# Thefefe/orbit

Hardware: AMD Instinct MI355X
Metric: meshlets_culled_per_sec (higher is better)
Workload: dtype f32

## Files before the change

orbit_amd/csrc/block_pretest.h:

```cpp
#pragma once
#include <math.h>
#include <stdint.h>
#include <string.h>

#if defined(__HIPCC__) || defined(__CUDACC__)
#define ORBIT_BLK_FN __host__ __device__ inline
#else
#define ORBIT_BLK_FN inline
#endif

namespace orbit {

ORBIT_BLK_FN uint32_t blk_bits(float f) {
    uint32_t u;
    __builtin_memcpy(&u, &f, 4);
    return u;
}
ORBIT_BLK_FN float blk_float(uint32_t u) {
    float f;
    __builtin_memcpy(&f, &u, 4);
    return f;
}
ORBIT_BLK_FN uint32_t blk_up16(float x) { return (blk_bits(x) + 0xFFFFu) >> 16; }

struct BlockBound {
    float cx, cy, cz;
    uint32_t packed;
    float rc;
    float r_max;
    uint32_t valid;
    uint32_t pad_;
};
static_assert(sizeof(BlockBound) == 32, "BlockBound layout");

ORBIT_BLK_FN BlockBound block_bound_unpack(float cx, float cy, float cz, uint32_t packed) {
    BlockBound b;
    b.cx = cx, b.cy = cy, b.cz = cz, b.packed = packed;
    b.rc = blk_float(packed & 0xFFFF0000u);
    b.r_max = blk_float(packed << 16);
    b.valid = (packed >> 16) != 0u ? 1u : 0u;
    b.pad_ = 0u;
    return b;
}

struct BlockRecord {
    float gx, gy, gz, dk;
    float sigma;
    float bk;
    float rr;
    uint32_t flags;
};
static_assert(sizeof(BlockRecord) == 32, "BlockRecord layout");
constexpr uint32_t kBlkSparse = 1u;
constexpr uint32_t kBlkInside = 2u;

constexpr float kBlkEps = 0x1p-18f;
constexpr float kBlkSlack = 1.0f + 0x1p-10f;
constexpr float kBlkUp = 1.0f + 0x1p-20f;
constexpr float kBlkTiny = 0x1p-80f;
constexpr float kBlkHuge = 0x1p60f;
#ifndef ORBIT_BLK_RATIO
#define ORBIT_BLK_RATIO 8.0f
#endif

ORBIT_BLK_FN float blk_max(float a, float b) { return a > b ? a : b; }

ORBIT_BLK_FN BlockBound block_bound_finish(float cx, float cy, float cz, float dist_max, float r_max, float r_min, bool finite) {
    BlockBound b;
    b.cx = cx, b.cy = cy, b.cz = cz;
    b.rc = dist_max * kBlkUp + 0x1p-60f;
    b.r_max = r_max;
    const bool ok = finite && r_min >= 0.0f && b.rc < kBlkHuge && r_max < kBlkHuge && fabsf(cx) < kBlkHuge &&
                    fabsf(cy) < kBlkHuge && fabsf(cz) < kBlkHuge;
    b.valid = ok ? 1u : 0u;
    b.packed = ok ? (blk_up16(b.rc) << 16 | blk_up16(r_max)) : 0u;
    b.pad_ = 0u;
    return b;
}
ORBIT_BLK_FN float block_dist(float cx, float cy, float cz, float x, float y, float z) {
    const float dx = x - cx, dy = y - cy, dz = z - cz;
    return sqrtf(fmaf(dz, dz, fmaf(dy, dy, dx * dx)));
}

ORBIT_BLK_FN BlockBound block_bound_of(const float *spheres, uint32_t n) {
    const float inf = INFINITY;
    float lo[3] = {inf, inf, inf}, hi[3] = {-inf, -inf, -inf}, r_max = 0.0f, r_min = 0.0f;
    bool finite = true;
    for (uint32_t i = 0; i < n; i++) {
        const float *s = spheres + 4 * i;
        for (int k = 0; k < 3; k++) lo[k] = fminf(lo[k], s[k]), hi[k] = fmaxf(hi[k], s[k]);
        r_max = fmaxf(r_max, s[3]), r_min = fminf(r_min, s[3]);
        finite = finite && isfinite(s[0]) && isfinite(s[1]) && isfinite(s[2]) && isfinite(s[3]);
    }
    const float cx = 0.5f * lo[0] + 0.5f * hi[0], cy = 0.5f * lo[1] + 0.5f * hi[1], cz = 0.5f * lo[2] + 0.5f * hi[2];
    float dist = 0.0f;
    for (uint32_t i = 0; i < n; i++) dist = fmaxf(dist, block_dist(cx, cy, cz, spheres[4 * i], spheres[4 * i + 1], spheres[4 * i + 2]));
    return block_bound_finish(cx, cy, cz, dist, r_max, r_min, finite);
}

ORBIT_BLK_FN BlockRecord block_record_setup(const float *m, bool affine, float scale, const BlockBound &b, bool covered,
                                            const float *planes, uint32_t n_planes, float ratio = ORBIT_BLK_RATIO) {
    BlockRecord o;
    const float Cx = b.cx, Cy = b.cy, Cz = b.cz;
    const float dx = fmaf(m[8], Cz, fmaf(m[4], Cy, fmaf(m[0], Cx, m[12])));
    const float dy = fmaf(m[9], Cz, fmaf(m[5], Cy, fmaf(m[1], Cx, m[13])));
    const float dz = fmaf(m[10], Cz, fmaf(m[6], Cy, fmaf(m[2], Cx, m[14])));
    const float aCx = fabsf(Cx), aCy = fabsf(Cy), aCz = fabsf(Cz);
    const float apx = fmaf(fabsf(m[8]), aCz, fmaf(fabsf(m[4]), aCy, fmaf(fabsf(m[0]), aCx, fabsf(m[12]))));
    const float apy = fmaf(fabsf(m[9]), aCz, fmaf(fabsf(m[5]), aCy, fmaf(fabsf(m[1]), aCx, fabsf(m[13]))));
    const float apz = fmaf(fabsf(m[10]), aCz, fmaf(fabsf(m[6]), aCy, fmaf(fabsf(m[2]), aCx, fabsf(m[14]))));
    const float g00 = fmaf(m[2], m[2], fmaf(m[1], m[1], m[0] * m[0]));
    const float g11 = fmaf(m[6], m[6], fmaf(m[5], m[5], m[4] * m[4]));
    const float g22 = fmaf(m[10], m[10], fmaf(m[9], m[9], m[8] * m[8]));
    const float g01 = fabsf(fmaf(m[2], m[6], fmaf(m[1], m[5], m[0] * m[4])));
    const float g02 = fabsf(fmaf(m[2], m[10], fmaf(m[1], m[9], m[0] * m[8])));
    const float g12 = fabsf(fmaf(m[6], m[10], fmaf(m[5], m[9], m[4] * m[8])));
    const float s2 = blk_max(g00 + g01 + g02, blk_max(g11 + g01 + g12, g22 + g02 + g12));
    const float sigma = sqrtf(s2) * (1.0f + 0x1p-16f) + 0x1p-60f;
    const float ap = (blk_max(apx, blk_max(apy, apz)) + 2.0f * sigma * b.rc) * kBlkUp;
    const float rcp = fmaf(kBlkEps, ap, sigma * b.rc * kBlkUp);
    const float D = sqrtf(fmaf(dz, dz, fmaf(dy, dy, dx * dx)));
    const float gx = fmaf(m[2], dz, fmaf(m[1], dy, m[0] * dx));
    const float gy = fmaf(m[6], dz, fmaf(m[5], dy, m[4] * dx));
    const float gz = fmaf(m[10], dz, fmaf(m[9], dy, m[8] * dx));
    const float kf = 0x1.020408p-7f;
    const float mag = ap + D + rcp;
    o.gx = gx * kf, o.gy = gy * kf, o.gz = gz * kf, o.dk = D * kf;
    o.sigma = sigma;
    o.bk = kf * fmaf(kBlkEps, mag, rcp) * kBlkSlack;
    o.rr = b.r_max * scale * kBlkSlack + kBlkTiny;
    bool sparse = affine && covered && b.valid != 0u && D > ratio * rcp && D > 0x1p-40f && mag < kBlkHuge &&
                  sigma < 0x1p40f && o.rr < kBlkHuge && scale >= 0.0f;
    bool inside = sparse;
    for (uint32_t i = 0; i < n_planes; i++) {
        const float nx = planes[4 * i], ny = planes[4 * i + 1], nz = planes[4 * i + 2], w = planes[4 * i + 3];
        const float nn = sqrtf(fmaf(nz, nz, fmaf(ny, ny, nx * nx))) * kBlkUp + kBlkTiny;
        const float dist = fmaf(nz, dz, fmaf(ny, dy, fmaf(nx, dx, w))) - nn * rcp;
        const float margin = fmaf(kBlkEps, fmaf(nn, mag, fabsf(w)), kBlkTiny);
        inside = inside && dist > margin;
    }
    o.flags = (sparse ? kBlkSparse : 0u) | (inside ? kBlkInside : 0u);
    return o;
}

ORBIT_BLK_FN void block_pretest_terms(const BlockRecord &r, uint32_t cone, float &s0, float &band) {
    const float ax = (float)(int)(int8_t)(cone & 0xFFu), ay = (float)(int)(int8_t)((cone >> 8) & 0xFFu);
    const float az = (float)(int)(int8_t)((cone >> 16) & 0xFFu), co = (float)(int)(int8_t)(cone >> 24);
    s0 = fmaf(r.gx, ax, fmaf(r.gy, ay, fmaf(r.gz, az, -(co * r.dk))));
    const float a1 = fabsf(ax) + fabsf(ay) + fabsf(az);
    band = fmaf(r.bk, fmaf(r.sigma, a1, fabsf(co)), kBlkTiny);
}
ORBIT_BLK_FN bool block_cone_culls(const BlockRecord &r, float s0, float band) { return s0 >= band + r.rr; }
ORBIT_BLK_FN bool block_cone_keeps(float s0, float band) { return s0 < -band; }
ORBIT_BLK_FN uint32_t block_pretest(const BlockRecord &r, uint32_t cone) {
    float s0, band;
    block_pretest_terms(r, cone, s0, band);
    return block_cone_culls(r, s0, band) ? 1u : (block_cone_keeps(s0, band) ? 2u : 0u);
}

}
```

orbit_amd/csrc/meshlet_eval_blocks.hip:

```cpp
#include "block_pretest.h"
#include "meshlet_common.h"

namespace orbit {

namespace {

constexpr int kBkWaves = 4;
constexpr int kBkWavesPerSimd = 5;
constexpr uint32_t kBkRing = 512, kBkFlush = 64;

struct __attribute__((aligned(16))) BlockTileLds {
    BlockRecord r[kTileRecords];
};
struct CandRing {
    uint16_t code[kBkRing];
};
struct RingState {
    uint32_t head = 0, count = 0;
    uint32_t total = 0;
};

__device__ __forceinline__ bool row_is_sparse(const WaveTileLds &L, int r) {
    const uint32_t w = reinterpret_cast<const uint32_t *>(&L.pad_)[0];
    return (((uint32_t)__builtin_amdgcn_readfirstlane((int)w) >> (2 * r)) & 1u) != 0u;
}

struct BoundRegs {
    float4 q;
};
__device__ __forceinline__ BoundRegs blk_load_bound(const MeshletCullParams &p, const BlockBound *blk, const uint4 &rec, int lane) {
    const int src_lane = (lane & 15) * 4;
    const uint32_t y = (uint32_t)__shfl((int)rec.y, src_lane, 64), z = (uint32_t)__shfl((int)rec.z, src_lane, 64);
    const uint32_t rel = y - p.ms.first;
    BoundRegs b;
    const bool covered = lane < (int)kTileRecords && z != 0u && (y & 31u) == 0u && rel < p.ms.count && z <= p.ms.count - rel;
    const float4 *src = covered ? reinterpret_cast<const float4 *>(blk + (y >> 5)) : reinterpret_cast<const float4 *>(p.zero_page);
    b.q = src[0];
    return b;
}

__device__ __forceinline__ void blk_setup(const MeshletCullParams &p, WaveTileLds &L, BlockTileLds &B, const PlaneLds &P,
                                          const BoundRegs &bb, int lane) {
    uint32_t flags = 0u;
    if (lane < (int)kTileRecords) {
        const RecordLds &R = L.r[lane];
        float m[16];
#pragma unroll
        for (int c = 0; c < 4; c++) {
            const float4 col = R.mcol[c];
            m[4 * c] = col.x, m[4 * c + 1] = col.y, m[4 * c + 2] = col.z, m[4 * c + 3] = col.w;
        }
        const BlockBound b = block_bound_unpack(bb.q.x, bb.q.y, bb.q.z, __float_as_uint(bb.q.w));
        const uint32_t aw = reinterpret_cast<const uint32_t *>(&L.affine_rows)[lane >> 3];
        const bool affine = ((aw >> (8 * ((lane >> 1) & 3))) & 1u) != 0u;
        BlockRecord o = block_record_setup(m, affine, R.scale, b, true, reinterpret_cast<const float *>(P.plane),
                                           min(p.ci.cull_plane_count, (uint32_t)ORBIT_MAX_CULL_PLANES));
        if (R.rec.z == 0u) o.flags = kBlkSparse;
        B.r[lane] = o;
        flags = o.flags;
    }
    uint64_t m = __ballot((flags & kBlkSparse) != 0u);
    m &= m >> 1;
    if (lane == 0) L.pad_ = m & 0x5555ull;
    __builtin_amdgcn_fence(__ATOMIC_RELEASE, "wavefront");
    __builtin_amdgcn_wave_barrier();
    __builtin_amdgcn_fence(__ATOMIC_ACQUIRE, "wavefront");
}

struct PipeRegs {
    uint32_t v[10];
};

__device__ __forceinline__ bool tile_is_sparse(const WaveTileLds &L) {
    const uint32_t w = reinterpret_cast<const uint32_t *>(&L.pad_)[0];
    return (uint32_t)__builtin_amdgcn_readfirstlane((int)w) == 0x5555u;
}

template <int R>
__device__ __forceinline__ void blk_row_load(const MeshletCullParams &p, const WaveTileLds &L, bool sparse, int lane,
                                             uint32_t *v, const StreamRsrc &SR) {
    const uint32_t half = lane >> 5, ml = lane & 31;
    const uint4 rec = L.r[2 * R + half].rec;
    const bool active = ml < rec.z;
    const uint32_t rel = rec.y + ml - SR.first;
    const bool in = active & (rel < SR.count);
    if (active & !in) latch_status(p.status, ORBIT_E_RANGE);
    const uint32_t i = in ? rel : kNoOffset >> 4;
    const uint32_t is = sparse ? kNoOffset >> 4 : i;
    const auto sp = __builtin_amdgcn_raw_buffer_load_b128(SR.sphere, is << 4, 0, ORBIT_EVAL_LOAD_AUX);
    v[4] = __builtin_amdgcn_raw_buffer_load_b32(SR.cone, i << 2, 0, ORBIT_EVAL_LOAD_AUX);
    v[0] = sp[0], v[1] = sp[1], v[2] = sp[2], v[3] = sp[3];
}

__device__ __forceinline__ void blk_tile_load(const MeshletCullParams &p, const WaveTileLds &L, int lane, uint32_t *v,
                                              const StreamRsrc &SR) {
    const uint32_t half = lane >> 5, ml = lane & 31;
    bool bad = false;
#pragma unroll
    for (int r = 0; r < (int)kTileRows; r++) {
        const uint4 rec = L.r[2 * r + half].rec;
        const bool active = ml < rec.z;
        const uint32_t rel = rec.y + ml - SR.first;
        const bool in = active & (rel < SR.count);
        bad |= active & !in;
        const uint32_t i = in ? rel : kNoOffset >> 4;
        v[r] = __builtin_amdgcn_raw_buffer_load_b32(SR.cone, i << 2, 0, ORBIT_EVAL_LOAD_AUX);
    }
    if (bad) latch_status(p.status, ORBIT_E_RANGE);
}

template <int R>
__device__ __forceinline__ uint32_t blk_row_dense(const MeshletCullParams &p, WaveTileLds &L, const PlaneLds &P, int lane,
                                                  const uint32_t *v, uint32_t total) {
    RowRegs<1> t;
    t.a[0] = make_uint4(v[0], v[1], v[2], v[3]);
    t.b[0] = make_uint4(v[4], 0u, 0u, 0u);
    t.prev[0] = 0u;
    return rows_eval<0, 0, R, 1, true>(p, L, P, nullptr, lane, t, total, nullptr);
}

template <int R>
__device__ __forceinline__ void blk_row_eval(WaveTileLds &L, const BlockTileLds &B, CandRing &ring, int lane,
                                             uint32_t cone, RingState &rs) {
    const uint32_t half = lane >> 5;
    const BlockRecord br = B.r[2 * R + half];
    float s0, band;
    block_pretest_terms(br, cone, s0, band);
    const uint64_t culled = ballot(block_cone_culls(br, s0, band));
    const uint64_t kept = ballot(block_cone_keeps(s0, band)) & ballot((br.flags & kBlkInside) != 0u);
    const uint32_t lo = (uint32_t)__builtin_amdgcn_readfirstlane((int)L.r[2 * R].amask.x);
    const uint32_t hi = (uint32_t)__builtin_amdgcn_readfirstlane((int)L.r[2 * R + 1].amask.x);
    const uint64_t allow = (uint64_t)hi << 32 | lo;
    const uint64_t draw = allow & kept & ~culled;
    const uint64_t cand = allow & ~culled & ~kept;
    if (lane == 0) L.draw_mask[R] = draw;
    rs.total += (uint32_t)__popcll(draw);
    if (lane_of(cand)) ring.code[(rs.head + rs.count + lane_prefix(cand)) & (kBkRing - 1u)] = (uint16_t)(R * 64 + lane);
    rs.count += (uint32_t)__popcll(cand);
}

__device__ __forceinline__ void blk_flush(const MeshletCullParams &p, WaveTileLds &L, const PlaneLds &P, const CandRing &ring,
                                          const StreamRsrc &SR, int lane, RingState &rs, uint32_t n) {
    __builtin_amdgcn_fence(__ATOMIC_RELEASE, "wavefront");
    __builtin_amdgcn_wave_barrier();
    __builtin_amdgcn_fence(__ATOMIC_ACQUIRE, "wavefront");
    const bool valid = (uint32_t)lane < n;
    const uint32_t code = valid ? (uint32_t)ring.code[(rs.head + (uint32_t)lane) & (kBkRing - 1u)] : 0u;
    const uint32_t rid = (code >> 5) & 15u, ml = code & 31u;
    const uint4 rec = L.r[rid].rec;
    const uint32_t rel = rec.y + ml - SR.first;
    const uint32_t i = (valid && ml < rec.z && rel < SR.count) ? rel : kNoOffset >> 4;
    const auto sp = __builtin_amdgcn_raw_buffer_load_b128(SR.sphere, i << 4, 0, 0);
    const uint32_t c = __builtin_amdgcn_raw_buffer_load_b32(SR.cone, i << 2, 0, 0);
    Sphere s;
    const uint64_t geo = eval_geometry_mask<0>(p, L, P, rid, make_uint4(sp[0], sp[1], sp[2], sp[3]), make_uint4(c, 0u, 0u, 0u), s, true);
    const uint64_t vis = geo & ballot(valid);
    if (lane_of(vis)) atomicOr(reinterpret_cast<uint32_t *>(L.draw_mask) + rid, 1u << ml);
    rs.total += (uint32_t)__popcll(vis);
    rs.head = (rs.head + n) & (kBkRing - 1u);
    rs.count -= n;
}

__global__ __launch_bounds__(kBkWaves * 64, kBkWavesPerSimd) void meshlet_eval_blocks_kernel(const MeshletCullParams p,
                                                                                            const BlockBound *blk) {
    __shared__ WaveTileLds lds[kBkWaves][3];
    __shared__ BlockTileLds blds[kBkWaves][2];
    __shared__ PlaneLds planes;
    __shared__ CandRing rings[kBkWaves];
    __shared__ uint32_t cls_sel[8];
    const int lane = threadIdx.x & 63, wave = __builtin_amdgcn_readfirstlane((int)(threadIdx.x >> 6));
    const uint32_t nrec_raw = *reinterpret_cast<const uint32_t *>(p.dispatch_buffer);
    const uint32_t stride = gridDim.x * kBkWaves, wave_g = (uint32_t)__builtin_amdgcn_readfirstlane((int)(blockIdx.x * kBkWaves + wave));
    const uint32_t cap_tiles = (p.dispatch_capacity + kTileRecords - 1) / kTileRecords;
    uint4 r0 = setup_load_rec(p, wave_g, wave_g < cap_tiles, p.dispatch_capacity, lane);
    uint4 r1 = setup_load_rec(p, wave_g + stride, wave_g + stride < cap_tiles, p.dispatch_capacity, lane);
    uint4 rec2 = setup_load_rec(p, wave_g + 2u * stride, wave_g + 2u * stride < cap_tiles, p.dispatch_capacity, lane);
    planes_to_lds(p, planes);
    clear_chunk_sums(p, kBkWaves * 64);
    if (threadIdx.x < 6) cls_sel[threadIdx.x] = ((alpha_bits(p.ci, threadIdx.x >> 1) >> (threadIdx.x & 1u)) & 1u) ? ~0u : 0u;
    __syncthreads();
    const uint32_t nrec = min(nrec_raw, p.dispatch_capacity);
    const uint32_t ntiles = (nrec + kTileRecords - 1) / kTileRecords;
    const uint32_t full_rounds = ntiles / stride;
    const uint32_t dyn_rounds = min(max(full_rounds / 4u, 1u), 3u);
    const uint32_t n_static = ntiles <= stride ? 0xFFFFFFFFu : max(full_rounds >= dyn_rounds ? full_rounds - dyn_rounds : 0u, 3u);
    const uint32_t npools = min((uint32_t)kTicketPools, stride);
    const uint32_t pool = wave_g % npools;
    uint32_t *ticket_ctr = p.tickets + pool * kTicketStride;
    uint32_t claims = 0;
    auto claim = [&]() -> uint32_t {
        uint32_t raw = claims;
        if (claims >= n_static) {
            raw = 0;
            if (lane == 0) raw = atomicAdd(ticket_ctr, 1u);
        }
        claims++;
        return raw;
    };
    auto ticket_tile = [&](uint32_t raw, uint32_t k) -> uint32_t {
        const uint32_t t = (uint32_t)__builtin_amdgcn_readfirstlane((int)raw);
        if (k < n_static) return t * stride + wave_g;
        return t >= 0x08000000u ? 0xFFFFFFFFu : n_static * stride + t * npools + pool;
    };
    StreamRsrc SR = {};
    SR.first = p.ms.first;
    SR.count = p.ms.count;
    SR.sphere = __builtin_amdgcn_make_buffer_rsrc(const_cast<uint4 *>(p.ms.sphere + p.ms.first), 0, p.ms.count * 16u, kBufFlags);
    SR.cone = __builtin_amdgcn_make_buffer_rsrc(const_cast<uint32_t *>(p.ms.cone + p.ms.first), 0, p.ms.count * 4u, kBufFlags);
    uint32_t w0, w1, w2, tk_raw;
    {
        const uint32_t t0 = claim(), t1 = claim(), t2 = claim();
        tk_raw = claim();
        w0 = ticket_tile(t0, 0u);
        w1 = ticket_tile(t1, 1u);
        w2 = ticket_tile(t2, 2u);
    }
    PipeRegs q;
    bool whole;
    uint32_t *const qa = q.v, *const qb = q.v + 5;
    {
        const uint4 none = make_uint4(0u, 0u, 0u, 0u);
        const uint32_t rl = (uint32_t)lane >> 2;
        if (!(w0 < ntiles && w0 * kTileRecords + rl < nrec)) r0 = none;
        if (!(w1 < ntiles && w1 * kTileRecords + rl < nrec)) r1 = none;
        if (!(w2 < ntiles && w2 * kTileRecords + rl < nrec)) rec2 = none;
        if ((lane & 3) == 0) lds[wave][0].r[lane >> 2].rec = r0;
        __builtin_amdgcn_fence(__ATOMIC_RELEASE, "wavefront");
        __builtin_amdgcn_wave_barrier();
        __builtin_amdgcn_fence(__ATOMIC_ACQUIRE, "wavefront");
        const float4 m0 = setup_load_mat(p, r0, lane);
        const float4 m1 = setup_load_mat(p, r1, lane);
        const uint32_t c0 = setup_load_cls(p, r0, lane), c1 = setup_load_cls(p, r1, lane);
        const BoundRegs b0 = blk_load_bound(p, blk, r0, lane), b1 = blk_load_bound(p, blk, r1, lane);
        setup_write_cls(lds[wave][0], cls_sel, r0, c0, lane);
        setup_write_cls(lds[wave][1], cls_sel, r1, c1, lane);
        setup_write(p, lds[wave][0], r0, m0, lane);
        blk_setup(p, lds[wave][0], blds[wave][0], planes, b0, lane);
        whole = tile_is_sparse(lds[wave][0]);
        if (whole) {
            blk_tile_load(p, lds[wave][0], lane, q.v, SR);
            q.v[8] = q.v[9] = 0u;
        } else {
            blk_row_load<0>(p, lds[wave][0], row_is_sparse(lds[wave][0], 0), lane, qa, SR);
            blk_row_load<1>(p, lds[wave][0], row_is_sparse(lds[wave][0], 1), lane, qb, SR);
        }
        setup_write(p, lds[wave][1], r1, m1, lane);
        blk_setup(p, lds[wave][1], blds[wave][1], planes, b1, lane);
    }
    uint32_t it = 0;
    const uint32_t prio_rank = blockIdx.x / max(gridDim.x / (uint32_t)kBkWavesPerSimd, 1u);
    while (w0 < ntiles) {
        switch ((it + prio_rank) & 3u) {
        case 0: __builtin_amdgcn_s_setprio(0); break;
        case 1: __builtin_amdgcn_s_setprio(1); break;
        case 2: __builtin_amdgcn_s_setprio(2); break;
        default: __builtin_amdgcn_s_setprio(3); break;
        }
        const uint32_t w3 = ticket_tile(tk_raw, claims - 1u);
        tk_raw = claim();
        WaveTileLds &L = lds[wave][it % 3];
        WaveTileLds &Ln = lds[wave][(it + 1) % 3];
        const BlockTileLds &B = blds[wave][it & 1u];
        CandRing &ring = rings[wave];
        RingState rs;
        const bool nxt_whole = tile_is_sparse(Ln);
        float4 mat2;
        uint32_t cls2;
        BoundRegs bnd2;
        uint4 rec3;
#define BK_FLUSH() \
    while (rs.count >= kBkFlush) blk_flush(p, L, planes, ring, SR, lane, rs, kBkFlush);
        if (whole) {
            PipeRegs tn;
            if (nxt_whole) {
                blk_tile_load(p, Ln, lane, tn.v, SR);
                tn.v[8] = tn.v[9] = 0u;
            } else {
                blk_row_load<0>(p, Ln, row_is_sparse(Ln, 0), lane, tn.v, SR);
                blk_row_load<1>(p, Ln, row_is_sparse(Ln, 1), lane, tn.v + 5, SR);
            }
            mat2 = setup_load_mat(p, rec2, lane);
            cls2 = setup_load_cls(p, rec2, lane);
            bnd2 = blk_load_bound(p, blk, rec2, lane);
            rec3 = setup_load_rec(p, w3, w3 < ntiles, nrec, lane);
            blk_row_eval<0>(L, B, ring, lane, q.v[0], rs);
            blk_row_eval<1>(L, B, ring, lane, q.v[1], rs);
            BK_FLUSH()
            blk_row_eval<2>(L, B, ring, lane, q.v[2], rs);
            blk_row_eval<3>(L, B, ring, lane, q.v[3], rs);
            BK_FLUSH()
            blk_row_eval<4>(L, B, ring, lane, q.v[4], rs);
            blk_row_eval<5>(L, B, ring, lane, q.v[5], rs);
            blk_row_eval<6>(L, B, ring, lane, q.v[6], rs);
            blk_row_eval<7>(L, B, ring, lane, q.v[7], rs);
            q = tn;
        } else {
#define BK_ROW(R, Q)                                                                                                   \
    if (row_is_sparse(L, R)) blk_row_eval<R>(L, B, ring, lane, (Q)[4], rs);                                            \
    else rs.total = blk_row_dense<R>(p, L, planes, lane, Q, rs.total);
            BK_ROW(0, qa)
            blk_row_load<2>(p, L, row_is_sparse(L, 2), lane, qa, SR);
            BK_ROW(1, qb)
            blk_row_load<3>(p, L, row_is_sparse(L, 3), lane, qb, SR);
            BK_FLUSH()
            BK_ROW(2, qa)
            blk_row_load<4>(p, L, row_is_sparse(L, 4), lane, qa, SR);
            BK_ROW(3, qb)
            blk_row_load<5>(p, L, row_is_sparse(L, 5), lane, qb, SR);
            BK_FLUSH()
            mat2 = setup_load_mat(p, rec2, lane);
            cls2 = setup_load_cls(p, rec2, lane);
            bnd2 = blk_load_bound(p, blk, rec2, lane);
            rec3 = setup_load_rec(p, w3, w3 < ntiles, nrec, lane);
            BK_ROW(4, qa)
            blk_row_load<6>(p, L, row_is_sparse(L, 6), lane, qa, SR);
            BK_ROW(5, qb)
            blk_row_load<7>(p, L, row_is_sparse(L, 7), lane, qb, SR);
            BK_ROW(6, qa)
            if (!nxt_whole) blk_row_load<0>(p, Ln, row_is_sparse(Ln, 0), lane, qa, SR);
            BK_ROW(7, qb)
            if (nxt_whole) {
                blk_tile_load(p, Ln, lane, q.v, SR);
                q.v[8] = q.v[9] = 0u;
            } else {
                blk_row_load<1>(p, Ln, row_is_sparse(Ln, 1), lane, qb, SR);
            }
#undef BK_ROW
        }
#undef BK_FLUSH
        whole = nxt_whole;
        setup_write_cls(lds[wave][(it + 2) % 3], cls_sel, rec2, cls2, lane);
        setup_write(p, lds[wave][(it + 2) % 3], rec2, mat2, lane);
        blk_setup(p, lds[wave][(it + 2) % 3], blds[wave][it & 1u], planes, bnd2, lane);
        while (rs.count > 0u) blk_flush(p, L, planes, ring, SR, lane, rs, min(rs.count, kBkFlush));
        __builtin_amdgcn_fence(__ATOMIC_RELEASE, "wavefront");
        __builtin_amdgcn_wave_barrier();
        __builtin_amdgcn_fence(__ATOMIC_ACQUIRE, "wavefront");
        if (lane < 2 * (int)kTileRows)
            p.tile_masks[(size_t)w0 * (2 * kTileRows) + lane] = reinterpret_cast<const uint32_t *>(L.draw_mask)[lane];
        if (lane == 0) p.tile_counts[w0] = rs.total;
        w0 = w1;
        w1 = w2;
        w2 = w3;
        rec2 = rec3;
        it++;
    }
}

}

hipError_t launch_meshlet_eval_blocks(const MeshletCullParams &p, const BlockBound *blk, dim3 grid, hipStream_t s) {
    hipLaunchKernelGGL(meshlet_eval_blocks_kernel, grid, dim3(kBkWaves * 64), 0, s, p, blk);
    return hipGetLastError();
}

}
```

orbit_amd/host/orbit_host_c.cpp:

```cpp
#include "orbit_host_c.h"

#include <cstring>
#include <map>
#include <memory>
#include <string>

#include "orbit_host.hpp"
#include "orbit_assets.hpp"
#include "orbit_gltf.hpp"
#include "orbit_raster.hpp"
#include "orbit_scene.hpp"
#include "../csrc/block_pretest.h"

using namespace orbit;
using namespace orbit::passes;

namespace {
thread_local std::string g_err = "no error";

struct HostCtx {
    std::unique_ptr<graphics::Context> ctx;
    std::map<std::string, std::unique_ptr<DepthPyramid>> pyramids;
};

// ... 526 lines not shown
int32_t orbit_host_raster_depth(const void *draw_commands, uint32_t max_commands, const uint32_t *meshlet_data,
                                uint64_t meshlet_data_words, const void *vertices, uint64_t vertex_count,
                                uint32_t vertex_stride, uint32_t position_offset, const OrbitEntityData *entity_data,
                                uint32_t entity_count, const float view_proj[16], float *depth, uint32_t width,
                                uint32_t height, uint32_t flags, OrbitRasterStats *stats, int32_t *command_error) {
    return guarded([&] {
        raster::HostJob j;
        j.draw_commands = (const uint32_t *)draw_commands, j.max_commands = max_commands;
        j.meshlet_data = meshlet_data, j.meshlet_data_words = meshlet_data_words;
        j.vertices = (const uint8_t *)vertices, j.vertex_count = vertex_count;
        j.vertex_stride = vertex_stride, j.position_offset = position_offset;
        j.entity_data = entity_data, j.entity_count = entity_count;
        j.view_proj = view_proj, j.depth = depth, j.width = width, j.height = height, j.flags = flags;
        raster::raster_depth(j, stats, command_error);
    });
}

int32_t orbit_host_raster_visibility(const void *draw_commands, uint32_t max_commands, const uint32_t *meshlet_data,
                                     uint64_t meshlet_data_words, const void *vertices, uint64_t vertex_count,
                                     uint32_t vertex_stride, uint32_t position_offset, const OrbitEntityData *entity_data,
                                     uint32_t entity_count, const float view_proj[16], uint64_t *visibility, uint32_t width,
                                     uint32_t height, uint32_t flags, uint32_t command_base, OrbitRasterStats *stats,
                                     int32_t *command_error) {
    return guarded([&] {
        raster::HostJob j;
        j.draw_commands = (const uint32_t *)draw_commands, j.max_commands = max_commands;
        j.meshlet_data = meshlet_data, j.meshlet_data_words = meshlet_data_words;
        j.vertices = (const uint8_t *)vertices, j.vertex_count = vertex_count;
        j.vertex_stride = vertex_stride, j.position_offset = position_offset;
        j.entity_data = entity_data, j.entity_count = entity_count;
        j.view_proj = view_proj, j.depth = nullptr, j.width = width, j.height = height, j.flags = flags;
        raster::raster_visibility(j, visibility, command_base, stats, command_error);
    });
}

int32_t orbit_host_visibility_resolve(const uint64_t *visibility, uint32_t width, uint32_t height, uint32_t command_base,
                                      uint32_t max_commands, float *depth, uint32_t *command_pixels,
                                      OrbitVisibilityStats *stats) {
    return guarded([&] {
        raster::visibility_resolve(visibility, width, height, command_base, max_commands, depth, command_pixels, stats);
    });
}

int32_t orbit_host_visibility_compact(const OrbitVisibilityCompact *job, int32_t *status) {
    return guarded([&] {
        if (!job) throw Panic("visibility_compact: job is NULL");
        raster::visibility_compact(*job, status);
    });
}

int32_t orbit_host_visibility_surface(const OrbitVisibilitySurface *job, int32_t *status) {
    return guarded([&] {
        if (!job) throw Panic("visibility_surface: job is NULL");
        raster::visibility_surface(*job, status);
    });
}

int32_t orbit_host_visibility_surface_drawn(const OrbitVisibilitySurface *job, uint32_t raster_flags, int32_t *status) {
    return guarded([&] {
        if (!job) throw Panic("visibility_surface_drawn: job is NULL");
        raster::visibility_surface_drawn(*job, raster_flags, status);
    });
}

void *orbit_host_gltf_load(const char *path) {
    gltf_loader::LoadedScene *scene = nullptr;
    const int32_t rc = guarded([&] {
        if (!path) throw Panic("path is NULL");
        auto s = std::make_unique<gltf_loader::LoadedScene>();
        std::string err;
        if (!gltf_loader::load_gltf(path, *s, err)) throw Panic("load_gltf: " + err);
        scene = s.release();
    });
    return rc == 0 ? scene : nullptr;
}
void orbit_host_gltf_free(void *scene) { delete static_cast<gltf_loader::LoadedScene *>(scene); }
void orbit_host_gltf_counts(const void *scene, OrbitHostGltfCounts *out) {
    const auto &s = *static_cast<const gltf_loader::LoadedScene *>(scene);
    out->meshes = s.assets.mesh_infos.size();
    out->meshlets = s.assets.meshlets.size();
    out->meshlet_data_words = s.assets.meshlet_data.size();
    out->materials = s.assets.materials.size();
    out->vertices = s.assets.vertex_positions.size() / 3;
    out->entities = s.entities.size();
}
const OrbitMeshInfo *orbit_host_gltf_mesh_infos(const void *scene) {
    return static_cast<const gltf_loader::LoadedScene *>(scene)->assets.mesh_infos.data();
}
const OrbitMeshlet *orbit_host_gltf_meshlets(const void *scene) {
    return static_cast<const gltf_loader::LoadedScene *>(scene)->assets.meshlets.data();
}
const uint32_t *orbit_host_gltf_meshlet_data(const void *scene) {
    return static_cast<const gltf_loader::LoadedScene *>(scene)->assets.meshlet_data.data();
}
const OrbitMaterialData *orbit_host_gltf_materials(const void *scene) {
    return static_cast<const gltf_loader::LoadedScene *>(scene)->assets.materials.data();
}
const float *orbit_host_gltf_vertex_positions(const void *scene) {
    return static_cast<const gltf_loader::LoadedScene *>(scene)->assets.vertex_positions.data();
}
uint64_t orbit_host_gltf_entities(const void *scene, OrbitHostGltfEntity *out, uint64_t capacity) {
    const auto &s = *static_cast<const gltf_loader::LoadedScene *>(scene);
    for (size_t i = 0; i < s.entities.size() && i < capacity; i++) {
        const auto &e = s.entities[i];
        out[i].mesh = e.mesh;
        const float p[3] = {e.transform.position.x, e.transform.position.y, e.transform.position.z};
        const float q[4] = {e.transform.orientation.x, e.transform.orientation.y, e.transform.orientation.z,
                            e.transform.orientation.w};
        const float sc[3] = {e.transform.scale.x, e.transform.scale.y, e.transform.scale.z};
        std::memcpy(out[i].position, p, 12);
        std::memcpy(out[i].orientation, q, 16);
        std::memcpy(out[i].scale, sc, 12);
    }
    return s.entities.size();
}
uint64_t orbit_host_simplify_clustered(const float *positions, uint64_t vertex_count, const uint32_t *indices,
                                       uint64_t index_count, uint64_t target_index_count, uint32_t *out,
                                       uint64_t capacity, uint64_t *needed) {
    std::vector<uint32_t> r;
    assets::simplify_clustered(positions, (size_t)vertex_count, indices, (size_t)index_count,
                               (size_t)target_index_count, r);
    if (needed) *needed = r.size();
    const size_t n = std::min<size_t>(r.size(), (size_t)capacity) / 3 * 3;
    if (out && n) std::memcpy(out, r.data(), n * 4);
    return n;
}
void orbit_host_transform_from_mat4(const float matrix[16], float position[3], float orientation[4], float scale[3]) {
    const passes::Transform t = gltf_loader::transform_from_mat4(Mat4::from_cols_array(matrix));
    position[0] = t.position.x, position[1] = t.position.y, position[2] = t.position.z;
    orientation[0] = t.orientation.x, orientation[1] = t.orientation.y, orientation[2] = t.orientation.z;
    orientation[3] = t.orientation.w;
    scale[0] = t.scale.x, scale[1] = t.scale.y, scale[2] = t.scale.z;
}

void orbit_host_block_bounds(const float *spheres, uint64_t count, void *out) {
    orbit::BlockBound *o = static_cast<orbit::BlockBound *>(out);
    for (uint64_t b = 0; b * 32u < count; b++) o[b] = orbit::block_bound_of(spheres + 128u * b, (uint32_t)std::min<uint64_t>(32u, count - 32u * b));
}

uint32_t orbit_host_block_pretest(const float m[16], int32_t affine, float scale, const void *bound, const float *planes,
                                  uint32_t n_planes, float ratio, const uint32_t *cones, uint64_t count, uint8_t *verdicts) {
    orbit::BlockBound in;
    memcpy(&in, bound, sizeof(in));
    const orbit::BlockBound b = orbit::block_bound_unpack(in.cx, in.cy, in.cz, in.packed);
    const orbit::BlockRecord r = orbit::block_record_setup(m, affine != 0, scale, b, true, planes, n_planes, ratio < 0.0f ? ORBIT_BLK_RATIO : ratio);
    for (uint64_t i = 0; i < count; i++) {
        uint32_t v = (r.flags & orbit::kBlkSparse) ? orbit::block_pretest(r, cones[i]) : 0u;
        if (v == 2u && (r.flags & orbit::kBlkInside)) v |= 4u;
        verdicts[i] = (uint8_t)v;
    }
    return r.flags;
}

}
```

orbit_amd/host/orbit_host_c.h:

```cpp
#ifndef ORBIT_HOST_C_H
#define ORBIT_HOST_C_H
#include "../../include/orbit_abi_ext.h"
#ifdef __cplusplus
extern "C" {
#endif

#define ORBIT_HOST_PANIC (-100)

typedef struct OrbitHostProjection {
    uint32_t kind;
    float fov, half_width, near_clip, far_clip;
} OrbitHostProjection;

typedef struct OrbitHostCullInfo {
    float view_matrix[16];
    float view_space_cull_planes[16][4];
    uint32_t plane_count;
    OrbitHostProjection projection;
    uint32_t occlusion_kind;
    void *visibility_buffer;
    void *meshlet_visibility_buffer;
    float *depth_pyramid;
    uint32_t depth_pyramid_size[2];
    uint32_t noskip_alphamode;
// ... 41 lines not shown
void orbit_host_frustum_planes_from_matrix(const float m[16], float out[6][4], int32_t normalize);
uint32_t orbit_host_mip_levels_from_size(uint32_t max_size);
int32_t orbit_host_project_sphere_clip_space(const float sphere[4], float znear, float p00, float p11, float aabb[4]);
int32_t orbit_host_cull_info_to_gpu(const OrbitHostCullInfo *ci, OrbitGpuCullInfo *out);
typedef struct OrbitHostShadowCascadeIn {
    uint32_t shadow_resolution;
    float cascade_split_lambda, max_shadow_distance;
    uint32_t min_mesh_lod, max_mesh_lod;
    float lod_base, lod_step;
    float direction[4];
    float camera_position[3], camera_orientation[4];
    float camera_fov, camera_near_clip, camera_aspect_ratio;
    uint32_t cascade_index, frustum_culling;
} OrbitHostShadowCascadeIn;
int32_t orbit_host_shadow_cascade(const OrbitHostShadowCascadeIn *in, OrbitHostCullInfo *out_cull_info,
                                  float out_light_projection_matrix[16], float *out_world_size);
void orbit_host_cluster_settings_derive(const OrbitHostClusterSettings *s, float z_near, OrbitHostClusterDerived *out);

void orbit_host_compute_cluster_aabb(const float inverse_projection[16], const float screen_size[2], float tile_size_px,
                                     const float cluster_count[3], float z_near, float z_far, const float cluster_id[3],
                                     float out_min_max[6]);

void *orbit_host_context_create(int32_t device, void *stream, const OrbitCaps *caps);
void orbit_host_context_destroy(void *hctx);
int32_t orbit_host_sync_meshlet_stream(void *hctx, void *meshlet_buffer, uint64_t first, uint64_t count,
                                       uint64_t capacity);
int32_t orbit_host_sync_meshlet_stream_materials(void *hctx, void *materials_buffer, uint32_t material_count);
int32_t orbit_host_create_meshlet_dispatch_command(void *hctx, const char *name, const OrbitHostAssets *assets,
                                                   const OrbitHostScene *scene, const OrbitHostCullInfo *ci,
                                                   OrbitGpuCullInfo *out_cull_info, OrbitHostBuffer *out_dispatch);
int32_t orbit_host_create_meshlet_draw_commands(void *hctx, const char *name, const OrbitHostAssets *assets,
                                                const OrbitHostScene *scene, const OrbitHostCullInfo *ci,
                                                const OrbitHostBuffer *dispatch, OrbitHostBuffer *out_draws);
int32_t orbit_host_create_draw_commands(void *hctx, const char *name, const OrbitHostAssets *assets,
                                        const OrbitHostScene *scene, const OrbitHostCullInfo *ci,
                                        OrbitHostBuffer *out_draws);
int32_t orbit_host_depth_pyramid_update(void *hctx, const char *name, const float *depth, uint32_t width,
                                        uint32_t height, float **out_pyramid, uint32_t out_size_mips[3]);
int32_t orbit_host_compute_clusters(void *hctx, const OrbitHostClusterSettings *settings, const float view_matrix[16],
                                    const OrbitHostProjection *projection, float aspect_ratio, const float *depth,
                                    uint32_t depth_size[2], uint32_t samples, const OrbitHostScene *scene,
                                    OrbitHostClusterOut *out);

typedef struct OrbitHostArenaIndex {
    uint32_t generation, slot;
} OrbitHostArenaIndex;
void *orbit_host_arena_create(void);
void orbit_host_arena_destroy(void *arena);
OrbitHostArenaIndex orbit_host_arena_insert(void *arena, int64_t value);
int32_t orbit_host_arena_get(const void *arena, OrbitHostArenaIndex index, int64_t *out);
int32_t orbit_host_arena_remove(void *arena, OrbitHostArenaIndex index, int64_t *out);
int32_t orbit_host_arena_has_index(const void *arena, OrbitHostArenaIndex index);
uint64_t orbit_host_arena_len(const void *arena);
uint64_t orbit_host_arena_iter(const void *arena, OrbitHostArenaIndex *indices, int64_t *values, uint64_t capacity);
void *orbit_host_freelist_create(uint64_t size);
void orbit_host_freelist_destroy(void *alloc);
int32_t orbit_host_freelist_allocate(void *alloc, uint64_t size, OrbitHostArenaIndex *out_index,
                                     uint64_t out_range[2]);
void orbit_host_freelist_deallocate(void *alloc, OrbitHostArenaIndex index);
uint64_t orbit_host_freelist_blocks(const void *alloc, uint64_t *ranges, int32_t *is_free, uint64_t capacity);

typedef struct OrbitHostLight {
    float color[3], intensity;
    uint32_t kind;
    float param;
    uint32_t irradiance_map_index, prefiltered_map_index;
    uint32_t cast_shadows;
} OrbitHostLight;
typedef struct OrbitHostEntity {
    float position[3], orientation[4], scale[3];
    int32_t mesh;
    int32_t has_light;
    OrbitHostLight light;
    const char *name;
} OrbitHostEntity;
void *orbit_host_scene_create(uint64_t visibility_chunk_count);
void orbit_host_scene_destroy(void *scene);
int64_t orbit_host_scene_add_entity(void *scene, const OrbitHostEntity *entity);
int32_t orbit_host_scene_set_transform(void *scene, uint64_t entity, const float position[3],
                                       const float orientation[4], const float scale[3]);
int32_t orbit_host_scene_update(void *scene, const OrbitMeshInfo *mesh_infos, uint64_t mesh_info_count,
                                float luminance_cutoff, uint64_t frame_index);
const void *orbit_host_scene_entity_draws(const void *scene, uint64_t *count);
const OrbitEntityData *orbit_host_scene_entity_data(const void *scene, uint64_t *count);
const OrbitLightData *orbit_host_scene_light_data(const void *scene, uint64_t *count);
uint64_t orbit_host_scene_shadow_command_count(const void *scene);
int32_t orbit_host_scene_update_deferred(void *scene, const OrbitMeshInfo *mesh_infos, uint64_t mesh_info_count,
                                         float luminance_cutoff, uint64_t frame_index);
const OrbitEntityTransform *orbit_host_scene_transforms(const void *scene, uint64_t *count);
int64_t orbit_host_scene_instance_index(const void *scene, uint64_t entity);
int64_t orbit_host_scene_add_entities(void *scene, const OrbitSceneEntity *table, const OrbitEntityTransform *transforms,
                                      uint64_t count);
int32_t orbit_host_scene_set_mesh(void *scene, uint64_t entity, int32_t mesh);
int32_t orbit_host_scene_update_device(void *scene, const OrbitMeshInfo *mesh_infos, uint64_t mesh_info_count);
const OrbitSceneEntity *orbit_host_scene_entity_table(const void *scene, uint64_t *count);
uint64_t orbit_host_scene_shadow_orientations(const void *scene, float *orientations, uint64_t capacity);
int64_t orbit_host_scene_light_index(const void *scene, uint64_t entity);

int32_t orbit_host_compute_meshlets(const float *positions, uint64_t vertex_count, const uint32_t *indices,
                                    uint64_t index_count, uint32_t material, uint32_t vertex_offset,
                                    uint32_t data_offset_base, OrbitMeshlet *out_meshlets, uint32_t *out_meshlet_data,
                                    uint64_t *meshlet_count, uint64_t *meshlet_data_words);
void orbit_host_compute_mesh_bounds(const float *positions, uint64_t vertex_count, float aabb_min[3], float aabb_max[3],
                                    float bounding_sphere[4]);

int32_t orbit_host_meshlet_bounds(const OrbitMeshlet *meshlets, uint64_t meshlet_capacity, const uint32_t *indices,
                                  uint64_t first, uint64_t count, const uint32_t *meshlet_data, uint64_t meshlet_data_words,
                                  const void *vertices, uint64_t vertex_count, uint32_t vertex_stride,
                                  uint32_t position_offset, OrbitMeshletBoundsFull *out, int32_t *range_error,
                                  uint32_t *updates);

int32_t orbit_host_raster_depth(const void *draw_commands, uint32_t max_commands, const uint32_t *meshlet_data,
                                uint64_t meshlet_data_words, const void *vertices, uint64_t vertex_count,
                                uint32_t vertex_stride, uint32_t position_offset, const OrbitEntityData *entity_data,
                                uint32_t entity_count, const float view_proj[16], float *depth, uint32_t width,
                                uint32_t height, uint32_t flags, OrbitRasterStats *stats, int32_t *command_error);

int32_t orbit_host_raster_visibility(const void *draw_commands, uint32_t max_commands, const uint32_t *meshlet_data,
                                     uint64_t meshlet_data_words, const void *vertices, uint64_t vertex_count,
                                     uint32_t vertex_stride, uint32_t position_offset, const OrbitEntityData *entity_data,
                                     uint32_t entity_count, const float view_proj[16], uint64_t *visibility, uint32_t width,
                                     uint32_t height, uint32_t flags, uint32_t command_base, OrbitRasterStats *stats,
                                     int32_t *command_error);
int32_t orbit_host_visibility_resolve(const uint64_t *visibility, uint32_t width, uint32_t height, uint32_t command_base,
                                      uint32_t max_commands, float *depth, uint32_t *command_pixels,
                                      OrbitVisibilityStats *stats);
int32_t orbit_host_visibility_compact(const OrbitVisibilityCompact *job, int32_t *status);
int32_t orbit_host_visibility_surface(const OrbitVisibilitySurface *job, int32_t *status);
int32_t orbit_host_visibility_surface_drawn(const OrbitVisibilitySurface *job, uint32_t raster_flags, int32_t *status);

typedef struct OrbitHostGltfCounts {
    uint64_t meshes, meshlets, meshlet_data_words, materials, vertices, entities;
} OrbitHostGltfCounts;
typedef struct OrbitHostGltfEntity {
    int32_t mesh;
    float position[3], orientation[4], scale[3];
} OrbitHostGltfEntity;
void *orbit_host_gltf_load(const char *path);
void orbit_host_gltf_free(void *scene);
void orbit_host_gltf_counts(const void *scene, OrbitHostGltfCounts *out);
const OrbitMeshInfo *orbit_host_gltf_mesh_infos(const void *scene);
const OrbitMeshlet *orbit_host_gltf_meshlets(const void *scene);
const uint32_t *orbit_host_gltf_meshlet_data(const void *scene);
const OrbitMaterialData *orbit_host_gltf_materials(const void *scene);
const float *orbit_host_gltf_vertex_positions(const void *scene);
uint64_t orbit_host_gltf_entities(const void *scene, OrbitHostGltfEntity *out, uint64_t capacity);
uint64_t orbit_host_simplify_clustered(const float *positions, uint64_t vertex_count, const uint32_t *indices,
                                       uint64_t index_count, uint64_t target_index_count, uint32_t *out,
                                       uint64_t capacity, uint64_t *needed);
void orbit_host_transform_from_mat4(const float matrix[16], float position[3], float orientation[4], float scale[3]);
void orbit_host_block_bounds(const float *spheres, uint64_t count, void *out);
uint32_t orbit_host_block_pretest(const float m[16], int32_t affine, float scale, const void *bound, const float *planes,
                                  uint32_t n_planes, float ratio, const uint32_t *cones, uint64_t count, uint8_t *verdicts);
#ifdef __cplusplus
}
#endif
#endif
```

Measured before the change: 220.5 billion.

## Split block record setup across quad lanes and precompute plane norms

```diff
diff --git a/orbit_amd/csrc/block_pretest.h b/orbit_amd/csrc/block_pretest.h
--- a/orbit_amd/csrc/block_pretest.h
+++ b/orbit_amd/csrc/block_pretest.h
@@ -96,6 +96,10 @@
     float dist = 0.0f;
     for (uint32_t i = 0; i < n; i++) dist = fmaxf(dist, block_dist(cx, cy, cz, spheres[4 * i], spheres[4 * i + 1], spheres[4 * i + 2]));
     return block_bound_finish(cx, cy, cz, dist, r_max, r_min, finite);
+}
+
+ORBIT_BLK_FN float block_plane_norm(float nx, float ny, float nz) {
+    return sqrtf(fmaf(nz, nz, fmaf(ny, ny, nx * nx))) * kBlkUp + kBlkTiny;
 }
 
 ORBIT_BLK_FN BlockRecord block_record_setup(const float *m, bool affine, float scale, const BlockBound &b, bool covered,
@@ -134,12 +138,85 @@
     bool inside = sparse;
     for (uint32_t i = 0; i < n_planes; i++) {
         const float nx = planes[4 * i], ny = planes[4 * i + 1], nz = planes[4 * i + 2], w = planes[4 * i + 3];
-        const float nn = sqrtf(fmaf(nz, nz, fmaf(ny, ny, nx * nx))) * kBlkUp + kBlkTiny;
+        const float nn = block_plane_norm(nx, ny, nz);
         const float dist = fmaf(nz, dz, fmaf(ny, dy, fmaf(nx, dx, w))) - nn * rcp;
         const float margin = fmaf(kBlkEps, fmaf(nn, mag, fabsf(w)), kBlkTiny);
         inside = inside && dist > margin;
     }
     o.flags = (sparse ? kBlkSparse : 0u) | (inside ? kBlkInside : 0u);
+    return o;
+}
+
+ORBIT_BLK_FN int block_quad_col_a(int k) { return k == 3 ? 0 : k; }
+ORBIT_BLK_FN int block_quad_col_b(int k) { return k < 2 ? k + 1 : 2; }
+struct BlockQuadShare {
+    float d, ap, gd, go;
+};
+ORBIT_BLK_FN BlockQuadShare block_quad_share(const float row[4], const float a[3], const float b[3], float Cx, float Cy, float Cz) {
+    BlockQuadShare s;
+    s.d = fmaf(row[2], Cz, fmaf(row[1], Cy, fmaf(row[0], Cx, row[3])));
+    s.ap = fmaf(fabsf(row[2]), fabsf(Cz), fmaf(fabsf(row[1]), fabsf(Cy), fmaf(fabsf(row[0]), fabsf(Cx), fabsf(row[3]))));
+    s.gd = fmaf(a[2], a[2], fmaf(a[1], a[1], a[0] * a[0]));
+    s.go = fabsf(fmaf(a[2], b[2], fmaf(a[1], b[1], a[0] * b[0])));
+    return s;
+}
+struct BlockQuadSums {
+    float dx, dy, dz;
+    float apx, apy, apz;
+    float g00, g11, g22;
+    float g01, g12, g02;
+};
+struct BlockQuadTail {
+    float sigma, rcp, D, mag, bk, rr;
+    bool sparse;
+};
+constexpr float kBlkKf = 0x1.020408p-7f;
+ORBIT_BLK_FN BlockQuadTail block_quad_tail(const BlockQuadSums &q, bool affine, float scale, const BlockBound &b, bool covered,
+                                           float ratio) {
+    BlockQuadTail t;
+    const float s2 = blk_max(q.g00 + q.g01 + q.g02, blk_max(q.g11 + q.g01 + q.g12, q.g22 + q.g02 + q.g12));
+    t.sigma = sqrtf(s2) * (1.0f + 0x1p-16f) + 0x1p-60f;
+    const float ap = (blk_max(q.apx, blk_max(q.apy, q.apz)) + 2.0f * t.sigma * b.rc) * kBlkUp;
+    t.rcp = fmaf(kBlkEps, ap, t.sigma * b.rc * kBlkUp);
+    t.D = sqrtf(fmaf(q.dz, q.dz, fmaf(q.dy, q.dy, q.dx * q.dx)));
+    t.mag = ap + t.D + t.rcp;
+    t.bk = kBlkKf * fmaf(kBlkEps, t.mag, t.rcp) * kBlkSlack;
+    t.rr = b.r_max * scale * kBlkSlack + kBlkTiny;
+    t.sparse = affine && covered && b.valid != 0u && t.D > ratio * t.rcp && t.D > 0x1p-40f && t.mag < kBlkHuge &&
+               t.sigma < 0x1p40f && t.rr < kBlkHuge && scale >= 0.0f;
+    return t;
+}
+ORBIT_BLK_FN float block_quad_out(int k, const float a[3], const BlockQuadSums &q, const BlockQuadTail &t) {
+    const float g = fmaf(a[2], q.dz, fmaf(a[1], q.dy, a[0] * q.dx));
+    return (k == 3 ? t.D : g) * kBlkKf;
+}
+ORBIT_BLK_FN bool block_quad_plane(const float pl[4], float nn, const BlockQuadSums &q, const BlockQuadTail &t) {
+    const float dist = fmaf(pl[2], q.dz, fmaf(pl[1], q.dy, fmaf(pl[0], q.dx, pl[3]))) - nn * t.rcp;
+    const float margin = fmaf(kBlkEps, fmaf(nn, t.mag, fabsf(pl[3])), kBlkTiny);
+    return dist > margin;
+}
+ORBIT_BLK_FN BlockRecord block_record_setup_quad(const float *m, bool affine, float scale, const BlockBound &b, bool covered,
+                                                 const float *planes, const float *plane_nn, uint32_t n_planes,
+                                                 float ratio = ORBIT_BLK_RATIO) {
+    BlockQuadShare s[4];
+    for (int k = 0; k < 4; k++) {
+        const float row[4] = {m[k], m[4 + k], m[8 + k], m[12 + k]};
+        s[k] = block_quad_share(row, m + 4 * block_quad_col_a(k), m + 4 * block_quad_col_b(k), b.cx, b.cy, b.cz);
+    }
+    const BlockQuadSums q = {s[0].d,  s[1].d,  s[2].d,  s[0].ap, s[1].ap, s[2].ap,
+                             s[0].gd, s[1].gd, s[2].gd, s[0].go, s[1].go, s[3].go};
+    float out[4];
+    BlockQuadTail t[4];
+    bool pass = true;
+    for (int k = 0; k < 4; k++) {
+        t[k] = block_quad_tail(q, affine, scale, b, covered, ratio);
+        out[k] = block_quad_out(k, m + 4 * block_quad_col_a(k), q, t[k]);
+        for (uint32_t i = (uint32_t)k; i < n_planes; i += 4u) pass = block_quad_plane(planes + 4 * i, plane_nn[i], q, t[k]) && pass;
+    }
+    BlockRecord o;
+    o.gx = out[0], o.gy = out[1], o.gz = out[2], o.dk = out[3];
+    o.sigma = t[0].sigma, o.bk = t[0].bk, o.rr = t[0].rr;
+    o.flags = (t[0].sparse ? kBlkSparse : 0u) | (t[0].sparse && pass ? kBlkInside : 0u);
     return o;
 }
 
diff --git a/orbit_amd/csrc/meshlet_eval_blocks.hip b/orbit_amd/csrc/meshlet_eval_blocks.hip
--- a/orbit_amd/csrc/meshlet_eval_blocks.hip
+++ b/orbit_amd/csrc/meshlet_eval_blocks.hip
@@ -28,40 +28,62 @@
 struct BoundRegs {
     float4 q;
 };
-__device__ __forceinline__ BoundRegs blk_load_bound(const MeshletCullParams &p, const BlockBound *blk, const uint4 &rec, int lane) {
-    const int src_lane = (lane & 15) * 4;
-    const uint32_t y = (uint32_t)__shfl((int)rec.y, src_lane, 64), z = (uint32_t)__shfl((int)rec.z, src_lane, 64);
+__device__ __forceinline__ BoundRegs blk_load_bound(const MeshletCullParams &p, const BlockBound *blk, const uint4 &rec) {
+    const uint32_t y = rec.y, z = rec.z;
     const uint32_t rel = y - p.ms.first;
     BoundRegs b;
-    const bool covered = lane < (int)kTileRecords && z != 0u && (y & 31u) == 0u && rel < p.ms.count && z <= p.ms.count - rel;
+    const bool covered = z != 0u && (y & 31u) == 0u && rel < p.ms.count && z <= p.ms.count - rel;
     const float4 *src = covered ? reinterpret_cast<const float4 *>(blk + (y >> 5)) : reinterpret_cast<const float4 *>(p.zero_page);
     b.q = src[0];
     return b;
 }
 
+template <int K>
+__device__ __forceinline__ float quad_bcast(float x) {
+    return __uint_as_float((uint32_t)__builtin_amdgcn_update_dpp(0, (int)__float_as_uint(x), K * 0x55, 0xF, 0xF, false));
+}
+
 __device__ __forceinline__ void blk_setup(const MeshletCullParams &p, WaveTileLds &L, BlockTileLds &B, const PlaneLds &P,
-                                          const BoundRegs &bb, int lane) {
-    uint32_t flags = 0u;
-    if (lane < (int)kTileRecords) {
-        const RecordLds &R = L.r[lane];
-        float m[16];
-#pragma unroll
-        for (int c = 0; c < 4; c++) {
-            const float4 col = R.mcol[c];
-            m[4 * c] = col.x, m[4 * c + 1] = col.y, m[4 * c + 2] = col.z, m[4 * c + 3] = col.w;
-        }
-        const BlockBound b = block_bound_unpack(bb.q.x, bb.q.y, bb.q.z, __float_as_uint(bb.q.w));
-        const uint32_t aw = reinterpret_cast<const uint32_t *>(&L.affine_rows)[lane >> 3];
-        const bool affine = ((aw >> (8 * ((lane >> 1) & 3))) & 1u) != 0u;
-        BlockRecord o = block_record_setup(m, affine, R.scale, b, true, reinterpret_cast<const float *>(P.plane),
-                                           min(p.ci.cull_plane_count, (uint32_t)ORBIT_MAX_CULL_PLANES));
-        if (R.rec.z == 0u) o.flags = kBlkSparse;
-        B.r[lane] = o;
-        flags = o.flags;
-    }
-    uint64_t m = __ballot((flags & kBlkSparse) != 0u);
-    m &= m >> 1;
-    if (lane == 0) L.pad_ = m & 0x5555ull;
+                                          const float *plane_nn, const uint4 &rec, const BoundRegs &bb, int lane) {
+    const int rid = lane >> 2, k = lane & 3;
+    const RecordLds &R = L.r[rid];
+    const float *mf = reinterpret_cast<const float *>(R.mcol);
+    const float row[4] = {mf[k], mf[4 + k], mf[8 + k], mf[12 + k]};
+    const float4 ca = R.mcol[block_quad_col_a(k)], cb = R.mcol[block_quad_col_b(k)];
+    const float a[3] = {ca.x, ca.y, ca.z}, bcol[3] = {cb.x, cb.y, cb.z};
+    const BlockBound b = block_bound_unpack(bb.q.x, bb.q.y, bb.q.z, __float_as_uint(bb.q.w));
+    const BlockQuadShare s = block_quad_share(row, a, bcol, b.cx, b.cy, b.cz);
+    const BlockQuadSums q = {quad_bcast<0>(s.d),  quad_bcast<1>(s.d),  quad_bcast<2>(s.d),  quad_bcast<0>(s.ap),
+                             quad_bcast<1>(s.ap), quad_bcast<2>(s.ap), quad_bcast<0>(s.gd), quad_bcast<1>(s.gd),
+                             quad_bcast<2>(s.gd), quad_bcast<0>(s.go), quad_bcast<1>(s.go), quad_bcast<3>(s.go)};
+    const uint32_t aw = reinterpret_cast<const uint32_t *>(&L.affine_rows)[lane >> 5];
+    const bool affine = ((aw >> (8 * ((lane >> 3) & 3))) & 1u) != 0u;
+    const BlockQuadTail t = block_quad_tail(q, affine, R.scale, b, true, ORBIT_BLK_RATIO);
+    reinterpret_cast<float *>(&B.r[rid])[k] = block_quad_out(k, a, q, t);
+    const uint32_t n = min(p.ci.cull_plane_count, (uint32_t)ORBIT_MAX_CULL_PLANES);
+    bool pass = true;
+    for (uint32_t i0 = 0; i0 < n; i0 += 4u) {
+        const bool has = i0 + (uint32_t)k < n;
+        const uint32_t i = has ? i0 + (uint32_t)k : 0u;
+        const float4 pl4 = P.plane[i];
+        const float pl[4] = {pl4.x, pl4.y, pl4.z, pl4.w};
+        pass &= block_quad_plane(pl, plane_nn[i], q, t) | !has;
+    }
+    uint64_t in = ballot(pass);
+    in &= in >> 1;
+    in &= in >> 2;
+    const bool none = rec.z == 0u;
+    if (k == 0) {
+        const uint32_t flags = none ? kBlkSparse : (t.sparse ? kBlkSparse | (lane_of(in) ? kBlkInside : 0u) : 0u);
+        reinterpret_cast<float4 *>(&B.r[rid])[1] = make_float4(t.sigma, t.bk, t.rr, __uint_as_float(flags));
+    }
+    uint64_t m = ballot(t.sparse || none);
+    m &= m >> 4;
+    m &= 0x0101010101010101ull;
+    m = (m | m >> 6) & 0x0005000500050005ull;
+    m = (m | m >> 12) & 0x0000005500000055ull;
+    m = (m | m >> 24) & 0x5555ull;
+    if (lane == 0) L.pad_ = m;
     __builtin_amdgcn_fence(__ATOMIC_RELEASE, "wavefront");
     __builtin_amdgcn_wave_barrier();
     __builtin_amdgcn_fence(__ATOMIC_ACQUIRE, "wavefront");
@@ -92,21 +114,14 @@
     v[0] = sp[0], v[1] = sp[1], v[2] = sp[2], v[3] = sp[3];
 }
 
-__device__ __forceinline__ void blk_tile_load(const MeshletCullParams &p, const WaveTileLds &L, int lane, uint32_t *v,
-                                              const StreamRsrc &SR) {
+__device__ __forceinline__ void blk_tile_load(const WaveTileLds &L, int lane, uint32_t *v, const StreamRsrc &SR) {
     const uint32_t half = lane >> 5, ml = lane & 31;
-    bool bad = false;
 #pragma unroll
     for (int r = 0; r < (int)kTileRows; r++) {
         const uint4 rec = L.r[2 * r + half].rec;
-        const bool active = ml < rec.z;
-        const uint32_t rel = rec.y + ml - SR.first;
-        const bool in = active & (rel < SR.count);
-        bad |= active & !in;
-        const uint32_t i = in ? rel : kNoOffset >> 4;
+        const uint32_t i = ml < rec.z ? rec.y + ml - SR.first : kNoOffset >> 4;
         v[r] = __builtin_amdgcn_raw_buffer_load_b32(SR.cone, i << 2, 0, ORBIT_EVAL_LOAD_AUX);
     }
-    if (bad) latch_status(p.status, ORBIT_E_RANGE);
 }
 
 template <int R>
@@ -167,6 +182,7 @@
     __shared__ BlockTileLds blds[kBkWaves][2];
     __shared__ PlaneLds planes;
     __shared__ CandRing rings[kBkWaves];
+    __shared__ float plane_nn[ORBIT_MAX_CULL_PLANES];
     __shared__ uint32_t cls_sel[8];
     const int lane = threadIdx.x & 63, wave = __builtin_amdgcn_readfirstlane((int)(threadIdx.x >> 6));
     const uint32_t nrec_raw = *reinterpret_cast<const uint32_t *>(p.dispatch_buffer);
@@ -176,6 +192,10 @@
     uint4 r1 = setup_load_rec(p, wave_g + stride, wave_g + stride < cap_tiles, p.dispatch_capacity, lane);
     uint4 rec2 = setup_load_rec(p, wave_g + 2u * stride, wave_g + 2u * stride < cap_tiles, p.dispatch_capacity, lane);
     planes_to_lds(p, planes);
+    if (threadIdx.x < min(p.ci.cull_plane_count, (uint32_t)ORBIT_MAX_CULL_PLANES)) {
+        const float *pl = p.ci.cull_planes[threadIdx.x];
+        plane_nn[threadIdx.x] = block_plane_norm(pl[0], pl[1], pl[2]);
+    }
     clear_chunk_sums(p, kBkWaves * 64);
     if (threadIdx.x < 6) cls_sel[threadIdx.x] = ((alpha_bits(p.ci, threadIdx.x >> 1) >> (threadIdx.x & 1u)) & 1u) ? ~0u : 0u;
     __syncthreads();
@@ -231,21 +251,21 @@
         const float4 m0 = setup_load_mat(p, r0, lane);
         const float4 m1 = setup_load_mat(p, r1, lane);
         const uint32_t c0 = setup_load_cls(p, r0, lane), c1 = setup_load_cls(p, r1, lane);
-        const BoundRegs b0 = blk_load_bound(p, blk, r0, lane), b1 = blk_load_bound(p, blk, r1, lane);
+        const BoundRegs b0 = blk_load_bound(p, blk, r0), b1 = blk_load_bound(p, blk, r1);
         setup_write_cls(lds[wave][0], cls_sel, r0, c0, lane);
         setup_write_cls(lds[wave][1], cls_sel, r1, c1, lane);
         setup_write(p, lds[wave][0], r0, m0, lane);
-        blk_setup(p, lds[wave][0], blds[wave][0], planes, b0, lane);
+        blk_setup(p, lds[wave][0], blds[wave][0], planes, plane_nn, r0, b0, lane);
         whole = tile_is_sparse(lds[wave][0]);
         if (whole) {
-            blk_tile_load(p, lds[wave][0], lane, q.v, SR);
+            blk_tile_load(lds[wave][0], lane, q.v, SR);
             q.v[8] = q.v[9] = 0u;
         } else {
             blk_row_load<0>(p, lds[wave][0], row_is_sparse(lds[wave][0], 0), lane, qa, SR);
             blk_row_load<1>(p, lds[wave][0], row_is_sparse(lds[wave][0], 1), lane, qb, SR);
         }
         setup_write(p, lds[wave][1], r1, m1, lane);
-        blk_setup(p, lds[wave][1], blds[wave][1], planes, b1, lane);
+        blk_setup(p, lds[wave][1], blds[wave][1], planes, plane_nn, r1, b1, lane);
     }
     uint32_t it = 0;
     const uint32_t prio_rank = blockIdx.x / max(gridDim.x / (uint32_t)kBkWavesPerSimd, 1u);
@@ -273,7 +293,7 @@
         if (whole) {
             PipeRegs tn;
             if (nxt_whole) {
-                blk_tile_load(p, Ln, lane, tn.v, SR);
+                blk_tile_load(Ln, lane, tn.v, SR);
                 tn.v[8] = tn.v[9] = 0u;
             } else {
                 blk_row_load<0>(p, Ln, row_is_sparse(Ln, 0), lane, tn.v, SR);
@@ -281,7 +301,7 @@
             }
             mat2 = setup_load_mat(p, rec2, lane);
             cls2 = setup_load_cls(p, rec2, lane);
-            bnd2 = blk_load_bound(p, blk, rec2, lane);
+            bnd2 = blk_load_bound(p, blk, rec2);
             rec3 = setup_load_rec(p, w3, w3 < ntiles, nrec, lane);
             blk_row_eval<0>(L, B, ring, lane, q.v[0], rs);
             blk_row_eval<1>(L, B, ring, lane, q.v[1], rs);
@@ -310,7 +330,7 @@
             BK_FLUSH()
             mat2 = setup_load_mat(p, rec2, lane);
             cls2 = setup_load_cls(p, rec2, lane);
-            bnd2 = blk_load_bound(p, blk, rec2, lane);
+            bnd2 = blk_load_bound(p, blk, rec2);
             rec3 = setup_load_rec(p, w3, w3 < ntiles, nrec, lane);
             BK_ROW(4, qa)
             blk_row_load<6>(p, L, row_is_sparse(L, 6), lane, qa, SR);
@@ -320,7 +340,7 @@
             if (!nxt_whole) blk_row_load<0>(p, Ln, row_is_sparse(Ln, 0), lane, qa, SR);
             BK_ROW(7, qb)
             if (nxt_whole) {
-                blk_tile_load(p, Ln, lane, q.v, SR);
+                blk_tile_load(Ln, lane, q.v, SR);
                 q.v[8] = q.v[9] = 0u;
             } else {
                 blk_row_load<1>(p, Ln, row_is_sparse(Ln, 1), lane, qb, SR);
@@ -331,7 +351,7 @@
         whole = nxt_whole;
         setup_write_cls(lds[wave][(it + 2) % 3], cls_sel, rec2, cls2, lane);
         setup_write(p, lds[wave][(it + 2) % 3], rec2, mat2, lane);
-        blk_setup(p, lds[wave][(it + 2) % 3], blds[wave][it & 1u], planes, bnd2, lane);
+        blk_setup(p, lds[wave][(it + 2) % 3], blds[wave][it & 1u], planes, plane_nn, rec2, bnd2, lane);
         while (rs.count > 0u) blk_flush(p, L, planes, ring, SR, lane, rs, min(rs.count, kBkFlush));
         __builtin_amdgcn_fence(__ATOMIC_RELEASE, "wavefront");
         __builtin_amdgcn_wave_barrier();
diff --git a/orbit_amd/host/orbit_host_c.cpp b/orbit_amd/host/orbit_host_c.cpp
--- a/orbit_amd/host/orbit_host_c.cpp
+++ b/orbit_amd/host/orbit_host_c.cpp
@@ -702,4 +702,23 @@
     return r.flags;
 }
 
-}
+void orbit_host_block_record(const float m[16], int32_t affine, float scale, const void *bound, const float *planes,
+                             uint32_t n_planes, float ratio, int32_t quad, void *out) {
+    orbit::BlockBound in;
+    memcpy(&in, bound, sizeof(in));
+    const orbit::BlockBound b = orbit::block_bound_unpack(in.cx, in.cy, in.cz, in.packed);
+    const float rt = ratio < 0.0f ? ORBIT_BLK_RATIO : ratio;
+    orbit::BlockRecord r;
+    if (quad != 0) {
+        std::vector<float> nn(n_planes);
+        for (uint32_t i = 0; i < n_planes; i++) nn[i] = orbit::block_plane_norm(planes[4 * i], planes[4 * i + 1], planes[4 * i + 2]);
+        r = orbit::block_record_setup_quad(m, affine != 0, scale, b, true, planes, nn.data(), n_planes, rt);
+    } else {
+        r = orbit::block_record_setup(m, affine != 0, scale, b, true, planes, n_planes, rt);
+    }
+    memcpy(out, &r, sizeof(r));
+}
+
+float orbit_host_block_plane_norm(float nx, float ny, float nz) { return orbit::block_plane_norm(nx, ny, nz); }
+
+}
diff --git a/orbit_amd/host/orbit_host_c.h b/orbit_amd/host/orbit_host_c.h
--- a/orbit_amd/host/orbit_host_c.h
+++ b/orbit_amd/host/orbit_host_c.h
@@ -217,6 +217,9 @@
 void orbit_host_block_bounds(const float *spheres, uint64_t count, void *out);
 uint32_t orbit_host_block_pretest(const float m[16], int32_t affine, float scale, const void *bound, const float *planes,
                                   uint32_t n_planes, float ratio, const uint32_t *cones, uint64_t count, uint8_t *verdicts);
+void orbit_host_block_record(const float m[16], int32_t affine, float scale, const void *bound, const float *planes,
+                             uint32_t n_planes, float ratio, int32_t quad, void *out);
+float orbit_host_block_plane_norm(float nx, float ny, float nz);
 #ifdef __cplusplus
 }
 #endif
```

After: 228.0 billion, median of 6. 1.03x the previous value.
